# bdwsq1996/Effi-MVS-plus

Measured on NVIDIA B200. Metric: depth_maps_per_sec_1600x1184_5view, higher is better.
Workload: dtype hi+lo bf16 MMA x3, f32 accumulate (3-D regularization, fp32-grade) / f32 (warp, lookup, regression)

## Files before the change

effi-mvs-plus_b200/csrc/conv3d_tc.cu:

```cuda
#include <cuda_bf16.h>

#include <algorithm>
#include <cstdlib>
#include <cstring>
#include <vector>

#include "common.cuh"

namespace effimvs {
namespace {

constexpr int TILE_M = 128;
constexpr int SEG_VOX = 136;
constexpr int SEG_BYTES = SEG_VOX * 16;
constexpr int MAX_SEGS = 96;
constexpr int MAX_OPS = 160;
constexpr int MAX_BLOCKS = 56;
constexpr int MAX_PHASES = 8;
constexpr int ZSWEEP_R = 4;

enum { L_REG = 0, L_SPLIT = 1 };

struct ActLayout {
    int kind, planes, D, H, W;
// ... 352 lines not shown
            v = T.transposed ? w[((size_t)ci * T.cout + n) * 27 + tap] : w[((size_t)n * T.cin + ci) * 27 + tap];
        }
        __nv_bfloat16 hi = __float2bfloat16(v);
        dst[i] = lo ? __float2bfloat16(v - __bfloat162float(hi)) : hi;
    }
}

struct PackJobs { int n; PackTable T[8]; const float* w[8]; __nv_bfloat16* dst[8]; };
__global__ void pack_weights_multi_kernel(const __grid_constant__ PackJobs J) {
    const PackTable& T = J.T[blockIdx.y];
    const float* __restrict__ w = J.w[blockIdx.y];
    __nv_bfloat16* __restrict__ dst = J.dst[blockIdx.y];
    const int total = T.n_blocks * 2 * T.rows * 8;
    for (int i = blockIdx.x * blockDim.x + threadIdx.x; i < total; i += gridDim.x * blockDim.x) {
        const int kk = i & 7, row_all = (i >> 3) % T.rows, j = (i / (8 * T.rows)) & 1, blk = i / (16 * T.rows);
        const int row = T.stack > 1 ? row_all % T.brows : row_all;
        const bool lo = row >= T.N;
        const int n = lo ? row - T.N : row;
        const Block c = T.blk[blk];
        const int tap_bc = j ? c.tap1 : c.tap0, cb = j ? c.cb1 : c.cb0;
        const int tap = (T.stack > 1 && tap_bc >= 0) ? (T.stack - 1 - row_all / T.brows) * 9 + tap_bc : tap_bc;
        float v = 0.0f;
        if (tap >= 0 && n < T.cout) {
            const int ci = cb + kk;
            v = T.transposed ? w[((size_t)ci * T.cout + n) * 27 + tap] : w[((size_t)n * T.cin + ci) * 27 + tap];
        }
        __nv_bfloat16 hi = __float2bfloat16(v);
        dst[i] = lo ? __float2bfloat16(v - __bfloat162float(hi)) : hi;
    }
}

struct HaloJobs { int n; uint4* ptr[8]; ActLayout L[8]; int planes_before[9]; };
__global__ void zero_halo_kernel(const __grid_constant__ HaloJobs J, int B) {
    int job = 0;
    while (job + 1 < J.n && (int)blockIdx.x >= J.planes_before[job + 1]) ++job;
    const ActLayout& L = J.L[job];
    const int d = L.kind == L_SPLIT ? L.D / 2 : L.D, Pz = d + 2;
    const int local = blockIdx.x - J.planes_before[job];
    const int vol = local / Pz, zp = local - vol * Pz;
    uint4* __restrict__ base = J.ptr[job] + (long long)vol * L.vs;
    const uint4 zero = make_uint4(0, 0, 0, 0);
    const int tid = blockIdx.y * blockDim.x + threadIdx.x, nt = gridDim.y * blockDim.x;
    if (zp == 0) for (int i = tid; i < L.guard; i += nt) base[i] = zero;
    if (zp == Pz - 1) for (int i = tid; i < L.guard; i += nt) base[L.vs - L.guard + i] = zero;
    uint4* __restrict__ plane = base + L.guard + (long long)zp * L.zstride;
    if (zp == 0 || zp == Pz - 1) {
        for (int i = tid; i < (int)L.zstride; i += nt) plane[i] = zero;
    } else {
        for (int i = tid; i < L.Px; i += nt) { plane[i] = zero; plane[(long long)(L.Py - 1) * L.Px + i] = zero; }
        for (int y = 1 + tid; y < L.Py - 1; y += nt) { plane[(long long)y * L.Px] = zero; plane[(long long)y * L.Px + L.Px - 1] = zero; }
    }
}

constexpr int CIN1_X = 4;
template <int S>
__global__ void __launch_bounds__(128)
conv_cin1_kernel(const float* __restrict__ x, const float* __restrict__ w, const float* __restrict__ bias, int D, int H, int W,
                 const ActLayout OL, int plane, uint4* __restrict__ out) {
    __shared__ __align__(16) float sw[27 * 8 + 8];
    pdl_trigger();
    for (int i = threadIdx.x; i < 27 * 8; i += blockDim.x) sw[(i % 27) * 8 + i / 27] = w[i];
    if (threadIdx.x < 8) sw[216 + threadIdx.x] = bias[threadIdx.x];
    pdl_wait();
    __syncthreads();
    const int b = blockIdx.y;
    const int Ho = OL.H, Wo = OL.W;
    const int Wq = (Wo + CIN1_X - 1) / CIN1_X;
    const size_t o = (size_t)blockIdx.x * blockDim.x + threadIdx.x;
    if (o >= (size_t)D * Ho * Wq) return;
    const int ox0 = (int)(o % Wq) * CIN1_X, oy = (int)((o / Wq) % Ho), oz = (int)(o / ((size_t)Wq * Ho));
    constexpr int NIN = (CIN1_X - 1) * S + 3;
    float acc[CIN1_X][8];
#pragma unroll
    for (int i = 0; i < CIN1_X; ++i)
#pragma unroll
        for (int c = 0; c < 8; ++c) acc[i][c] = sw[216 + c];
    const float* xb = x + (size_t)b * D * H * W;
    const int ix0 = ox0 * S - 1;
#pragma unroll
    for (int a = 0; a < 3; ++a) {
        const int iz = oz + a - 1;
#pragma unroll
        for (int bb = 0; bb < 3; ++bb) {
            const int iy = oy * S + bb - 1;
            const bool row_ok = iz >= 0 && iz < D && iy >= 0 && iy < H;
            const float* row = xb + ((size_t)(row_ok ? iz : 0) * H + (row_ok ? iy : 0)) * W;
            float in[NIN];
#pragma unroll
            for (int j = 0; j < NIN; ++j) {
                const int ix = ix0 + j;
                in[j] = (row_ok && ix >= 0 && ix < W) ? __ldg(row + ix) : 0.0f;
            }
#pragma unroll
            for (int c = 0; c < 3; ++c) {
                const float4 w0 = *reinterpret_cast<const float4*>(sw + (a * 9 + bb * 3 + c) * 8);
                const float4 w1 = *reinterpret_cast<const float4*>(sw + (a * 9 + bb * 3 + c) * 8 + 4);
#pragma unroll
                for (int i = 0; i < CIN1_X; ++i) {
                    const float v = in[i * S + c];
                    acc[i][0] = fmaf(v, w0.x, acc[i][0]); acc[i][1] = fmaf(v, w0.y, acc[i][1]);
                    acc[i][2] = fmaf(v, w0.z, acc[i][2]); acc[i][3] = fmaf(v, w0.w, acc[i][3]);
                    acc[i][4] = fmaf(v, w1.x, acc[i][4]); acc[i][5] = fmaf(v, w1.y, acc[i][5]);
                    acc[i][6] = fmaf(v, w1.z, acc[i][6]); acc[i][7] = fmaf(v, w1.w, acc[i][7]);
                }
            }
        }
    }
#pragma unroll
    for (int i = 0; i < CIN1_X; ++i) {
        if (ox0 + i >= Wo) break;
#pragma unroll
        for (int j = 0; j < 8; ++j) acc[i][j] = fmaxf(acc[i][j], 0.0f);
        store_voxel(out, OL, b, plane, oz, oy, ox0 + i, acc[i]);
    }
}

__global__ void to_c8_kernel(const float* __restrict__ x, int C, const ActLayout L, uint4* __restrict__ out) {
    const int b = blockIdx.y;
    const int groups = (C + 7) / 8;
    const size_t vox = (size_t)L.D * L.H * L.W;
    const size_t o = (size_t)blockIdx.x * blockDim.x + threadIdx.x;
    if (o >= vox * groups) return;
    const int g = (int)(o / vox);
    const size_t r = o % vox;
    const int xx = (int)(r % L.W), yy = (int)((r / L.W) % L.H), zz = (int)(r / ((size_t)L.W * L.H));
    float v[8];
#pragma unroll
    for (int j = 0; j < 8; ++j) {
        const int c = g * 8 + j;
        v[j] = c < C ? x[((size_t)b * C + c) * vox + r] : 0.0f;
    }
    store_voxel(out, L, b, g, zz, yy, xx, v);
}
__global__ void from_c8_kernel(const uint4* __restrict__ in, int C, const ActLayout L, float* __restrict__ y) {
    const int b = blockIdx.y;
    const int groups = (C + 7) / 8;
    const size_t vox = (size_t)L.D * L.H * L.W;
    const size_t o = (size_t)blockIdx.x * blockDim.x + threadIdx.x;
    if (o >= vox * groups) return;
    const int g = (int)(o / vox);
    const size_t r = o % vox;
    const int xx = (int)(r % L.W), yy = (int)((r / L.W) % L.H), zz = (int)(r / ((size_t)L.W * L.H));
    float v[8];
    load_voxel(in, L, b, g, zz, yy, xx, v);
#pragma unroll
    for (int j = 0; j < 8; ++j) {
        const int c = g * 8 + j;
        if (c < C) y[((size_t)b * C + c) * vox + r] = v[j];
    }
}

struct Term { int seg, byte_off, tap, cls; };
struct PlaneSeg { long long off; int copy_vox; };

int pow2_cols(int n) { int c = 32; while (c < n) c <<= 1; return c; }

bool assemble(ConvProgram& P, PackTable& T, const std::vector<Term>& terms, const std::vector<PlaneSeg>& pseg, int NP,
              long long plane_stride, long long lo_plane_off, bool hilo) {
    const int SPP = (int)pseg.size();
    const int halves = hilo ? 2 : 1;
    const int n_phases = (hilo && NP == 4) ? 2 : 1;
    const int NPph = NP / n_phases;
    if (n_phases > MAX_PHASES) return false;
    P.n_phases = n_phases;
    P.b_rows = T.rows = hilo ? 2 * P.N : P.N;
    P.b_lbo_rows = P.b_rows; P.cls_z = 0; T.stack = 1; T.brows = T.rows;
// ... 243 lines not shown
int run_pack_multi(int n, const PackTable* T, const float* const* w, void* const* dst, cudaStream_t st) {
    static thread_local PackJobs J;
    J.n = n;
    int most = 0;
    for (int i = 0; i < n; ++i) {
        J.T[i] = T[i]; J.w[i] = w[i]; J.dst[i] = (__nv_bfloat16*)dst[i];
        most = std::max(most, T[i].n_blocks * 2 * T[i].rows * 8);
    }
    pack_weights_multi_kernel<<<dim3(ceil_div(most, 256), n), 256, 0, st>>>(J);
    return check_launch("pack_weights_multi_kernel");
}

int run_zero_halo(int n, void* const* ptr, const ActLayout* L, int B, cudaStream_t st) {
    static thread_local HaloJobs J;
    J.n = n;
    int total = 0;
    for (int i = 0; i < n; ++i) {
        J.ptr[i] = (uint4*)ptr[i]; J.L[i] = L[i];
        J.planes_before[i] = total;
        const int d = L[i].kind == L_SPLIT ? L[i].D / 2 : L[i].D;
        total += B * L[i].planes * (L[i].kind == L_SPLIT ? 8 : 1) * (d + 2);
    }
    J.planes_before[n] = total;
    zero_halo_kernel<<<dim3(total, 16), 128, 0, st>>>(J, B);
    return check_launch("zero_halo_kernel");
}

int run_tile_kernel(const ConvProgram& P, int B, const void* in, const ActLayout& IL, const void* wpk, const float* bias,
                    const ActLayout& OL, void* out, const ActLayout* RL, const void* res, float* out_f32, cudaStream_t st) {
    size_t smem = program_smem(P);
    EFFI_REQUIRE(smem <= 220 * 1024, EFFIMVS_EUNSUPPORTED, "conv_tc: tile needs %zu bytes of shared memory", smem);
    static bool attr_set = false;
    if (!attr_set) {
        cudaError_t e = cudaFuncSetAttribute(conv_tc_kernel, cudaFuncAttributeMaxDynamicSharedMemorySize, 220 * 1024);
        if (e != cudaSuccess) { set_error("conv_tc: cudaFuncSetAttribute: %s", cudaGetErrorString(e)); return EFFIMVS_ECUDA; }
        attr_set = true;
    }
    const int tiles_per_plane = ceil_div(P.gH * P.gPx, TILE_M);
    const long long n_tiles = (long long)tiles_per_plane * P.gD * B;
    EFFI_REQUIRE(n_tiles < (1ll << 31) && (long long)P.gPx * (P.gH + 2) < (1ll << 30), EFFIMVS_EUNSUPPORTED, "conv_tc: volume too large");
    int per_sm = (smem <= 110 * 1024 && P.tmem_cols <= 256) ? 2 : 1;
    if (const char* e = getenv("EFFIMVS_TC_MAXCTA")) {
        const int by_smem = (int)((227 * 1024) / (smem + 1024 + 4096)), by_tmem = 512 / P.tmem_cols;
        per_sm = std::max(1, std::min(atoi(e), std::min(by_smem, by_tmem)));
    }
    const int grid = (int)std::min<long long>(n_tiles, (long long)kNumSMs * per_sm);
    ActLayout rl = RL ? *RL : OL;
    if (const char* dbg = getenv("EFFIMVS_TC_DEBUG")) const_cast<ConvProgram&>(P).debug = atoi(dbg);
    launch_kernel(conv_tc_kernel, grid, dim3(CTA_THREADS), smem, st, P, (const uint4*)in, IL.batch_stride, (const uint8_t*)wpk, bias, OL, (uint4*)out, rl,
                                                    (const uint4*)res, out_f32, (int)n_tiles, tiles_per_plane);
    return check_launch("conv_tc_kernel");
}

int run_cin1(const float* x, const float* w, const float* bias, int B, int D, int H, int W, int s, const ActLayout& OL, int plane,
             void* out, cudaStream_t st) {
    size_t work = (size_t)D * OL.H * ((OL.W + CIN1_X - 1) / CIN1_X);
    dim3 grid((unsigned)((work + 127) / 128), B);
    if (s == 2) launch_kernel(conv_cin1_kernel<2>, grid, dim3(128), 0, st, x, w, bias, D, H, W, OL, plane, (uint4*)out);
    else launch_kernel(conv_cin1_kernel<1>, grid, dim3(128), 0, st, x, w, bias, D, H, W, OL, plane, (uint4*)out);
    return check_launch("conv_cin1_kernel");
}

template <bool RAW = false>
__device__ __forceinline__ void load_voxel_f32(const uint4* __restrict__ hi, long long lo_delta, long long idx, float (&v)[8]) {
    if (RAW) {
        const uint4 a = __ldg(hi + idx), c = __ldg(hi + idx + lo_delta);
        v[0] = __uint_as_float(a.x); v[1] = __uint_as_float(a.y); v[2] = __uint_as_float(a.z); v[3] = __uint_as_float(a.w);
        v[4] = __uint_as_float(c.x); v[5] = __uint_as_float(c.y); v[6] = __uint_as_float(c.z); v[7] = __uint_as_float(c.w);
        return;
    }
    unpack_bf16x8(__ldg(hi + idx), v);
    if (lo_delta) {
        float l[8];
        unpack_bf16x8(__ldg(hi + idx + lo_delta), l);
#pragma unroll
        for (int j = 0; j < 8; ++j) v[j] += l[j];
    }
}

constexpr int COUT1_X = 4;

template <bool RAW>
__global__ void __launch_bounds__(128)
conv_cout1_kernel(const uint4* __restrict__ in, const ActLayout IL, const float* __restrict__ w, const float* __restrict__ bias, int relu,
                  float* __restrict__ out) {
    __shared__ __align__(16) float sw[27 * 8];
    pdl_trigger();
    for (int i = threadIdx.x; i < 27 * 8; i += blockDim.x) sw[(i % 27) * 8 + i / 27] = w[i];
    pdl_wait();
    __syncthreads();
    const int b = blockIdx.y, D = IL.D, H = IL.H, W = IL.W;
    const int Wq = (W + COUT1_X - 1) / COUT1_X;
    const size_t o = (size_t)blockIdx.x * blockDim.x + threadIdx.x;
    if (o >= (size_t)D * H * Wq) return;
    const int x0 = (int)(o % Wq) * COUT1_X, y = (int)((o / Wq) % H), z = (int)(o / ((size_t)Wq * H));
    const long long lo_delta = (long long)IL.lo_off * IL.vs;
    const long long base = (long long)b * IL.batch_stride + IL.guard;
    float acc[COUT1_X];
#pragma unroll
    for (int i = 0; i < COUT1_X; ++i) acc[i] = bias ? __ldg(bias) : 0.0f;
#pragma unroll
    for (int a = 0; a < 3; ++a)
#pragma unroll
        for (int bb = 0; bb < 3; ++bb) {
            const long long row = base + (long long)(z + a) * IL.zstride + (long long)(y + bb) * IL.Px + x0;
            float v[COUT1_X + 2][8];
#pragma unroll
            for (int j = 0; j < COUT1_X + 2; ++j) {
                if (x0 + j <= W + 1) load_voxel_f32<RAW>(in, lo_delta, row + j, v[j]);
                else {
#pragma unroll
                    for (int c = 0; c < 8; ++c) v[j][c] = 0.0f;
                }
            }
#pragma unroll
            for (int c = 0; c < 3; ++c) {
                const float4 w0 = *reinterpret_cast<const float4*>(sw + (a * 9 + bb * 3 + c) * 8);
                const float4 w1 = *reinterpret_cast<const float4*>(sw + (a * 9 + bb * 3 + c) * 8 + 4);
#pragma unroll
                for (int i = 0; i < COUT1_X; ++i) {
                    const float (&u)[8] = v[i + c];
                    float t = acc[i];
                    t = fmaf(u[0], w0.x, t); t = fmaf(u[1], w0.y, t); t = fmaf(u[2], w0.z, t); t = fmaf(u[3], w0.w, t);
                    t = fmaf(u[4], w1.x, t); t = fmaf(u[5], w1.y, t); t = fmaf(u[6], w1.z, t); t = fmaf(u[7], w1.w, t);
                    acc[i] = t;
                }
            }
        }
    float* op = out + (((size_t)b * D + z) * H + y) * W + x0;
#pragma unroll
    for (int i = 0; i < COUT1_X; ++i)
        if (x0 + i < W) op[i] = relu ? fmaxf(acc[i], 0.0f) : acc[i];
}

template <bool RAW>
__global__ void __launch_bounds__(128)
deconv_cout1_kernel(const uint4* __restrict__ in, const ActLayout IL, const float* __restrict__ w, const float* __restrict__ bias, int relu,
                    float* __restrict__ out) {
    __shared__ __align__(16) float sw[27 * 8];
    pdl_trigger();
    for (int i = threadIdx.x; i < 27 * 8; i += blockDim.x) sw[(i % 27) * 8 + i / 27] = w[i];
    pdl_wait();
    __syncthreads();
    const int b = blockIdx.y, D = IL.D, H = IL.H, W = IL.W;
    const size_t o = (size_t)blockIdx.x * blockDim.x + threadIdx.x;
    if (o >= (size_t)D * H * W) return;
    const int x = (int)(o % W), y = (int)((o / W) % H), z = (int)(o / ((size_t)W * H));
    const long long lo_delta = (long long)IL.lo_off * IL.vs;
    const long long base = (long long)b * IL.batch_stride + IL.guard;
    const float b0 = bias ? __ldg(bias) : 0.0f;
    float acc[2][2] = {{b0, b0}, {b0, b0}};
    {
        const bool last = (threadIdx.x & 31) == 31 || x == W - 1;
#pragma unroll
        for (int a = 0; a < 3; ++a)
#pragma unroll
            for (int dy = 0; dy < 2; ++dy) {
                const uint4* p = in + base + (long long)(z + 2 - a) * IL.zstride + (long long)(y + 1 + dy) * IL.Px + (x + 1);
                asm volatile("prefetch.global.L1 [%0];" ::"l"(p));
                if (RAW || lo_delta) asm volatile("prefetch.global.L1 [%0];" ::"l"(p + lo_delta));
                if (last) {
                    asm volatile("prefetch.global.L1 [%0];" ::"l"(p + 1));
                    if (RAW || lo_delta) asm volatile("prefetch.global.L1 [%0];" ::"l"(p + 1 + lo_delta));
                }
            }
    }
    float v[3][2][2][8];
#pragma unroll
    for (int a = 0; a < 3; ++a) {
        const long long plane = base + (long long)(z + 2 - a) * IL.zstride;
#pragma unroll
        for (int dy = 0; dy < 2; ++dy)
#pragma unroll
            for (int dx = 0; dx < 2; ++dx) load_voxel_f32<RAW>(in, lo_delta, plane + (long long)(y + 1 + dy) * IL.Px + (x + 1 + dx), v[a][dy][dx]);
    }
#pragma unroll
    for (int a = 0; a < 3; ++a) {
#pragma unroll
        for (int bb = 0; bb < 3; ++bb)
#pragma unroll
            for (int c = 0; c < 3; ++c) {
                const int py = bb != 1, dy = bb == 0, px = c != 1, dx = c == 0;
                const float4 w0 = *reinterpret_cast<const float4*>(sw + (a * 9 + bb * 3 + c) * 8);
                const float4 w1 = *reinterpret_cast<const float4*>(sw + (a * 9 + bb * 3 + c) * 8 + 4);
                const float (&u)[8] = v[a][dy][dx];
                float t = acc[py][px];
                t = fmaf(u[0], w0.x, t); t = fmaf(u[1], w0.y, t); t = fmaf(u[2], w0.z, t); t = fmaf(u[3], w0.w, t);
                t = fmaf(u[4], w1.x, t); t = fmaf(u[5], w1.y, t); t = fmaf(u[6], w1.z, t); t = fmaf(u[7], w1.w, t);
                acc[py][px] = t;
            }
    }
    const int Ho = 2 * H, Wo = 2 * W;
#pragma unroll
    for (int py = 0; py < 2; ++py) {
        float2 r = make_float2(acc[py][0], acc[py][1]);
        if (relu) { r.x = fmaxf(r.x, 0.0f); r.y = fmaxf(r.y, 0.0f); }
        *reinterpret_cast<float2*>(out + (((size_t)b * D + z) * Ho + 2 * y + py) * Wo + 2 * x) = r;
    }
}

int run_cout1(bool deconv, int B, const void* in, const ActLayout& IL, const float* w, const float* bias, int relu, float* out,
              cudaStream_t st, bool raw_f32 = false) {
    if (deconv) {
        const size_t work = (size_t)IL.D * IL.H * IL.W;
        const dim3 grid((unsigned)((work + 127) / 128), B);
        if (raw_f32) launch_kernel(deconv_cout1_kernel<true>, grid, dim3(128), 0, st, (const uint4*)in, IL, w, bias, relu, out);
        else launch_kernel(deconv_cout1_kernel<false>, grid, dim3(128), 0, st, (const uint4*)in, IL, w, bias, relu, out);
        return check_launch("deconv_cout1_kernel");
    }
    const size_t work = (size_t)IL.D * IL.H * ((IL.W + COUT1_X - 1) / COUT1_X);
    const dim3 grid((unsigned)((work + 127) / 128), B);
    if (raw_f32) launch_kernel(conv_cout1_kernel<true>, grid, dim3(128), 0, st, (const uint4*)in, IL, w, bias, relu, out);
    else launch_kernel(conv_cout1_kernel<false>, grid, dim3(128), 0, st, (const uint4*)in, IL, w, bias, relu, out);
    return check_launch("conv_cout1_kernel");
}

struct Carver {
    char* base; size_t off, cap;
    void* take(size_t bytes) { void* p = base ? base + off : nullptr; off += (bytes + 255) & ~(size_t)255; return p; }
};

constexpr size_t W_SLOT = 128 * 1024;

}

size_t costreg_bf16_workspace_bytes(int B, int D, int H, int W, bool hilo) {
    ActLayout c0 = make_layout(L_REG, 8, D, H, W, hilo), c1 = make_layout(L_SPLIT, 8, D, H, W, hilo);
    ActLayout c2 = make_layout(L_REG, 16, D / 2, H / 2, W / 2, hilo), c3 = make_layout(L_SPLIT, 16, D / 2, H / 2, W / 2, hilo);
    ActLayout c4 = make_layout(L_REG, 32, D / 4, H / 4, W / 4, hilo);
    return layout_bytes(c0, B) * 2 + layout_bytes(c1, B) + layout_bytes(c2, B) * 2 + layout_bytes(c3, B) + layout_bytes(c4, B) * 2 +
           8 * W_SLOT + 4096;
}

int costreg_bf16(const float* x, const float* const* weights, const float* const* biases, int B, int D, int H, int W, bool hilo,
                 int phases, void* ws, size_t ws_bytes, float* prob_out, cudaStream_t st) {
    EFFI_REQUIRE(D % 4 == 0 && H % 4 == 0 && W % 4 == 0, EFFIMVS_EUNSUPPORTED, "costreg bf16: D, H, W must be multiples of 4");
    EFFI_REQUIRE(D <= 65535 && B <= 65535, EFFIMVS_EUNSUPPORTED, "costreg bf16: D or B too large");
    const int D2 = D / 2, H2 = H / 2, W2 = W / 2, D4 = D / 4, H4 = H / 4, W4 = W / 4;
    ActLayout L0 = make_layout(L_REG, 8, D, H, W, hilo), L1 = make_layout(L_SPLIT, 8, D, H, W, hilo);
    ActLayout L2 = make_layout(L_REG, 16, D2, H2, W2, hilo), L3 = make_layout(L_SPLIT, 16, D2, H2, W2, hilo);
    ActLayout L4 = make_layout(L_REG, 32, D4, H4, W4, hilo), L5 = L4, L6 = L2, L7 = L0;
    Carver cv{(char*)ws, 0, ws_bytes};
    void* c0 = cv.take(layout_bytes(L0, B)); void* c7 = cv.take(layout_bytes(L7, B)); void* c1 = cv.take(layout_bytes(L1, B));
    void* c2 = cv.take(layout_bytes(L2, B)); void* c6 = cv.take(layout_bytes(L6, B)); void* c3 = cv.take(layout_bytes(L3, B));
    void* c4 = cv.take(layout_bytes(L4, B)); void* c5 = cv.take(layout_bytes(L5, B));
    const size_t act_bytes = cv.off;
    void* wp[8];
    for (int i = 0; i < 8; ++i) wp[i] = cv.take(W_SLOT);
    EFFI_REQUIRE(cv.off <= ws_bytes, EFFIMVS_EWORKSPACE, "costreg bf16: workspace %zu < %zu", ws_bytes, cv.off);
    (void)act_bytes;
    int rc;
    const bool prepare = (phases & EFFIMVS_WS_PREPARE) != 0, run = (phases & EFFIMVS_WS_RUN) != 0;
    if (prepare) {
        void* bufs[8] = {c0, c7, c1, c2, c6, c3, c4, c5};
        ActLayout lays[8] = {L0, L7, L1, L2, L6, L3, L4, L5};
        if ((rc = run_zero_halo(8, bufs, lays, B, st))) return rc;
    }

    static thread_local ConvProgram P[8];
    static thread_local PackTable T[8];
    bool ok = build_conv_s1(P[0], T[0], 8, 8, L0, 1) && build_conv_s2(P[1], T[1], 8, 16, L1, 1) &&
              build_conv_s1(P[2], T[2], 16, 16, L2, 1) && build_conv_s2(P[3], T[3], 16, 32, L3, 1) &&
              build_conv_s1(P[4], T[4], 32, 32, L4, 1) && build_deconv(P[5], T[5], 32, 16, L5, 2, 1) &&
              build_deconv(P[6], T[6], 16, 8, L6, 2, 1) && build_conv_s1(P[7], T[7], 8, 1, L7, 0);
    EFFI_REQUIRE(ok, EFFIMVS_EUNSUPPORTED, "costreg bf16: program does not fit");
    for (int i = 0; i < 8; ++i)
        EFFI_REQUIRE(program_weight_bytes(T[i]) <= W_SLOT, EFFIMVS_EUNSUPPORTED, "costreg bf16: packed weights of layer %d too large", i + 1);
    if (prepare && (rc = run_pack_multi(8, T, weights + 1, wp, st))) return rc;
    if (!run) return EFFIMVS_OK;
    if ((rc = run_cin1(x, weights[0], biases[0], B, D, H, W, 1, L0, 0, c0, st))) return rc;
    if ((rc = run_tile_kernel(P[0], B, c0, L0, wp[0], biases[1], L1, c1, nullptr, nullptr, nullptr, st))) return rc;
    if ((rc = run_tile_kernel(P[1], B, c1, L1, wp[1], biases[2], L2, c2, nullptr, nullptr, nullptr, st))) return rc;
    if ((rc = run_tile_kernel(P[2], B, c2, L2, wp[2], biases[3], L3, c3, nullptr, nullptr, nullptr, st))) return rc;
    if ((rc = run_tile_kernel(P[3], B, c3, L3, wp[3], biases[4], L4, c4, nullptr, nullptr, nullptr, st))) return rc;
    if ((rc = run_tile_kernel(P[4], B, c4, L4, wp[4], biases[5], L5, c5, nullptr, nullptr, nullptr, st))) return rc;
    if ((rc = run_tile_kernel(P[5], B, c5, L5, wp[5], biases[6], L6, c6, &L3, c3, nullptr, st))) return rc;
    const char* prob_path = getenv("EFFIMVS_PROB_PATH");
    const bool raw_prob = hilo && prob_path && !strcmp(prob_path, "raw");
    P[6].out_f32_pair = raw_prob ? 1 : 0;
    if ((rc = run_tile_kernel(P[6], B, c6, L6, wp[6], biases[7], L7, c7, &L1, c1, nullptr, st))) return rc;
    if (raw_prob) return run_cout1(false, B, c7, L7, weights[8], nullptr, 0, prob_out, st, true);
    if (getenv("EFFIMVS_CUDA_CORE_PROB")) return run_cout1(false, B, c7, L7, weights[8], nullptr, 0, prob_out, st);
    return run_tile_kernel(P[7], B, c7, L7, wp[7], nullptr, L7, nullptr, nullptr, nullptr, prob_out, st);
}

size_t cost_up_bf16_workspace_bytes(int B, int D, int H, int W, bool hilo) {
    ActLayout cat = make_layout(L_REG, 16, D, H / 2, W / 2, hilo), c1 = make_layout(L_REG, 8, D, H / 2, W / 2, hilo);
    return layout_bytes(cat, B) + layout_bytes(c1, B) + 2 * W_SLOT + 4096;
}

int cost_up_bf16(const float* x, const float* prev, const float* const* weights, const float* const* biases, int B, int D, int H,
                 int W, bool hilo, int phases, void* ws, size_t ws_bytes, float* out, cudaStream_t st) {
    EFFI_REQUIRE(D <= 65535 && B <= 65535, EFFIMVS_EUNSUPPORTED, "cost_up bf16: D or B too large");
    const int H2 = H / 2, W2 = W / 2;
    ActLayout Lcat = make_layout(L_REG, 16, D, H2, W2, hilo), L1 = make_layout(L_REG, 8, D, H2, W2, hilo);
    Carver cv{(char*)ws, 0, ws_bytes};
    void* cat = cv.take(layout_bytes(Lcat, B)); void* c1 = cv.take(layout_bytes(L1, B));
    const size_t act_bytes = cv.off;
    void* wp1 = cv.take(W_SLOT); void* wp2 = cv.take(W_SLOT);
    EFFI_REQUIRE(cv.off <= ws_bytes, EFFIMVS_EWORKSPACE, "cost_up bf16: workspace %zu < %zu", ws_bytes, cv.off);
    (void)act_bytes;
    int rc;
    const bool prepare = (phases & EFFIMVS_WS_PREPARE) != 0, run = (phases & EFFIMVS_WS_RUN) != 0;
    if (prepare) {
        void* bufs[2] = {cat, c1};
        ActLayout lays[2] = {Lcat, L1};
        if ((rc = run_zero_halo(2, bufs, lays, B, st))) return rc;
    }
    static thread_local ConvProgram P1, P2;
    static thread_local PackTable T12[2];
    PackTable &T1 = T12[0], &T2 = T12[1];
    bool ok = build_conv_s1(P1, T1, 16, 8, Lcat, 1) && build_deconv(P2, T2, 8, 1, L1, 1, 1);
    EFFI_REQUIRE(ok, EFFIMVS_EUNSUPPORTED, "cost_up bf16: program does not fit");
    if (prepare) {
        void* dsts[2] = {wp1, wp2};
        if ((rc = run_pack_multi(2, T12, weights + 2, dsts, st))) return rc;
    }
    if (!run) return EFFIMVS_OK;
    if ((rc = run_cin1(x, weights[0], biases[0], B, D, H, W, 2, Lcat, 0, cat, st))) return rc;
    if ((rc = run_cin1(prev, weights[1], biases[1], B, D, H2, W2, 1, Lcat, 1, cat, st))) return rc;
    const bool tc_cout1 = getenv("EFFIMVS_TC_COUT1") != nullptr;
    const bool raw = hilo && !tc_cout1 && !getenv("EFFIMVS_NO_RAW_F32");
    P1.out_f32_pair = raw ? 1 : 0;
    if ((rc = run_tile_kernel(P1, B, cat, Lcat, wp1, biases[2], L1, c1, nullptr, nullptr, nullptr, st))) return rc;
    ActLayout LO = make_layout(L_REG, 8, D, H, W, false);
    if (!tc_cout1) return run_cout1(true, B, c1, L1, weights[3], biases[3], 1, out, st, raw);
    return run_tile_kernel(P2, B, c1, L1, wp2, biases[3], LO, nullptr, nullptr, nullptr, out, st);
}

size_t conv3d_bf16_workspace_bytes(int B, int Cin, int Cout, int D, int H, int W, int sd, int transposed, bool hilo) {
    int Do = D, Ho = H, Wo = W;
    if (transposed) { Do = D * sd; Ho = H * 2; Wo = W * 2; }
    else if (sd == 2) { Do = D / 2; Ho = H / 2; Wo = W / 2; }
    ActLayout LI = make_layout(!transposed && sd == 2 ? L_SPLIT : L_REG, (Cin + 7) / 8 * 8, D, H, W, hilo);
    ActLayout LO = make_layout(L_REG, (Cout + 7) / 8 * 8, Do, Ho, Wo, hilo);
    return layout_bytes(LI, B) + 2 * layout_bytes(LO, B) + W_SLOT + 4096;
}

int conv3d_bf16(const float* x, const float* weight, const float* bias, const float* residual, int B, int Cin, int Cout, int D,
                int H, int W, int sd, int transposed, int relu, bool hilo, void* ws, size_t ws_bytes, float* y, cudaStream_t st) {
    EFFI_REQUIRE((Cin == 8 || Cin == 16 || Cin == 32) && Cout >= 1 && Cout <= 32, EFFIMVS_EUNSUPPORTED,
                 "conv3d_bf16: Cin in {8,16,32}, Cout <= 32");
    int Do = D, Ho = H, Wo = W;
    if (transposed) { Do = D * sd; Ho = H * 2; Wo = W * 2; }
    else if (sd == 2) { EFFI_REQUIRE(D % 2 == 0 && H % 2 == 0 && W % 2 == 0, EFFIMVS_EUNSUPPORTED, "conv3d_bf16: stride 2 needs even dims"); Do = D / 2; Ho = H / 2; Wo = W / 2; }
    const int Cop = (Cout + 7) / 8 * 8;
    ActLayout LI = make_layout(!transposed && sd == 2 ? L_SPLIT : L_REG, Cin, D, H, W, hilo);
    ActLayout LO = make_layout(L_REG, Cop, Do, Ho, Wo, hilo);
    Carver cv{(char*)ws, 0, ws_bytes};
    void* xin = cv.take(layout_bytes(LI, B)); void* yout = cv.take(layout_bytes(LO, B)); void* rin = cv.take(layout_bytes(LO, B));
    const size_t act_bytes = cv.off;
    void* wp = cv.take(W_SLOT);
    EFFI_REQUIRE(cv.off <= ws_bytes, EFFIMVS_EWORKSPACE, "conv3d_bf16: workspace %zu < %zu", ws_bytes, cv.off);
    if (cudaMemsetAsync(ws, 0, act_bytes, st) != cudaSuccess) { set_error("conv3d_bf16: memset failed"); return EFFIMVS_ECUDA; }
    static thread_local ConvProgram P;
    static thread_local PackTable T;
    bool ok = transposed ? build_deconv(P, T, Cin, Cout, LI, sd, relu) : (sd == 2 ? build_conv_s2(P, T, Cin, Cout, LI, relu) : build_conv_s1(P, T, Cin, Cout, LI, relu));
    EFFI_REQUIRE(ok && program_weight_bytes(T) <= W_SLOT, EFFIMVS_EUNSUPPORTED, "conv3d_bf16: program does not fit");
    int rc;
    if ((rc = run_pack(T, weight, wp, st))) return rc;
    size_t n_in = (size_t)D * H * W * (Cin / 8), n_out = (size_t)Do * Ho * Wo * (Cop / 8);
    to_c8_kernel<<<dim3((unsigned)((n_in + 255) / 256), B), 256, 0, st>>>(x, Cin, LI, (uint4*)xin);
    if (residual) to_c8_kernel<<<dim3((unsigned)((n_out + 255) / 256), B), 256, 0, st>>>(residual, Cout, LO, (uint4*)rin);
    if ((rc = check_launch("to_c8_kernel"))) return rc;
    if ((rc = run_tile_kernel(P, B, xin, LI, wp, bias, LO, yout, residual ? &LO : nullptr, residual ? rin : nullptr, nullptr, st))) return rc;
    from_c8_kernel<<<dim3((unsigned)((n_out + 255) / 256), B), 256, 0, st>>>((const uint4*)yout, Cout, LO, y);
    return check_launch("from_c8_kernel");
}

}

extern "C" size_t effimvs_conv3d_bf16_workspace_bytes(int B, int Cin, int Cout, int D, int H, int W, int sd, int transposed, int precision) {
    return effimvs::conv3d_bf16_workspace_bytes(B, Cin, Cout, D, H, W, sd, transposed, precision == EFFIMVS_PREC_BF16X3);
// ... 11 lines not shown
```

Baseline: 165.7.

## Tile thin Cin=1 conv and Cout=1 deconv kernels with shared-memory z-ring reuse

Rewrites the single-input-channel conv kernel as a 2-D tiled kernel that sweeps along depth, staging input planes into a four-slot shared-memory ring with cp.async. Each loaded plane is reused across three output depths and neighbouring pixels instead of being re-read from global memory. Accumulation uses packed f32x2 FMAs, and the two cost_up cin1 launches are fused into one kernel that writes both planes. The Cout=1 deconv gets the same z-ring treatment with register-staged prefetch of the next plane, in exchange for more shared memory, a barrier per depth step, and fewer CTAs per SM.

```diff
diff --git a/effi-mvs-plus_b200/csrc/conv3d_tc.cu b/effi-mvs-plus_b200/csrc/conv3d_tc.cu
--- a/effi-mvs-plus_b200/csrc/conv3d_tc.cu
+++ b/effi-mvs-plus_b200/csrc/conv3d_tc.cu
@@ -428,66 +428,153 @@
     }
 }
 
-constexpr int CIN1_X = 4;
+constexpr int THIN_THREADS = 128;
+constexpr int THIN_RING = 4;
+
+int thin_zrun(int tiles, int B, int D) {
+    const int runs = std::min(D, std::max(1, ceil_div(4 * kNumSMs, tiles * B)));
+    return ceil_div(D, runs);
+}
+
+typedef unsigned long long pk2;
+__device__ __forceinline__ pk2 pk(float lo, float hi) { pk2 r; asm("mov.b64 %0, {%1, %2};" : "=l"(r) : "f"(lo), "f"(hi)); return r; }
+__device__ __forceinline__ void unpk(pk2 v, float& lo, float& hi) { asm("mov.b64 {%0, %1}, %2;" : "=f"(lo), "=f"(hi) : "l"(v)); }
+__device__ __forceinline__ void fma2_acc(pk2& acc, pk2 a, pk2 b) { asm("fma.rn.f32x2 %0, %1, %2, %0;" : "+l"(acc) : "l"(a), "l"(b)); }
+
+constexpr int CIN_TX = 64, CIN_TY = 8, CIN_PX = 4;
+static_assert(CIN_TX / CIN_PX * CIN_TY == THIN_THREADS, "one output row segment per thread");
 template <int S>
-__global__ void __launch_bounds__(128)
-conv_cin1_kernel(const float* __restrict__ x, const float* __restrict__ w, const float* __restrict__ bias, int D, int H, int W,
-                 const ActLayout OL, int plane, uint4* __restrict__ out) {
-    __shared__ __align__(16) float sw[27 * 8 + 8];
-    pdl_trigger();
-    for (int i = threadIdx.x; i < 27 * 8; i += blockDim.x) sw[(i % 27) * 8 + i / 27] = w[i];
-    if (threadIdx.x < 8) sw[216 + threadIdx.x] = bias[threadIdx.x];
-    pdl_wait();
-    __syncthreads();
-    const int b = blockIdx.y;
-    const int Ho = OL.H, Wo = OL.W;
-    const int Wq = (Wo + CIN1_X - 1) / CIN1_X;
-    const size_t o = (size_t)blockIdx.x * blockDim.x + threadIdx.x;
-    if (o >= (size_t)D * Ho * Wq) return;
-    const int ox0 = (int)(o % Wq) * CIN1_X, oy = (int)((o / Wq) % Ho), oz = (int)(o / ((size_t)Wq * Ho));
-    constexpr int NIN = (CIN1_X - 1) * S + 3;
-    float acc[CIN1_X][8];
-#pragma unroll
-    for (int i = 0; i < CIN1_X; ++i)
-#pragma unroll
-        for (int c = 0; c < 8; ++c) acc[i][c] = sw[216 + c];
-    const float* xb = x + (size_t)b * D * H * W;
-    const int ix0 = ox0 * S - 1;
-#pragma unroll
+struct CinRows {
+    static constexpr int ROWS = (CIN_TY - 1) * S + 3;
+    static constexpr int COLS = ((CIN_TX - 1) * S + 3 + 3) / 4 * 4;
+    static constexpr int PLANE = ROWS * COLS;
+    static constexpr int PER_THREAD = (PLANE + THIN_THREADS - 1) / THIN_THREADS;
+    static constexpr int NIN = (CIN_PX - 1) * S + 3;
+};
+
+template <int S>
+__device__ __forceinline__ void cin_stage(float* __restrict__ slot, const float* __restrict__ xb, int D, int H, int W, int z, int gy0,
+                                          int gx0) {
+    using R = CinRows<S>;
+    const bool zok = z >= 0 && z < D;
+    const float* __restrict__ pl = xb + (size_t)(zok ? z : 0) * H * W;
+#pragma unroll
+    for (int i = 0; i < R::PER_THREAD; ++i) {
+        const int e = threadIdx.x + i * THIN_THREADS;
+        if (e >= R::PLANE) break;
+        const int row = e / R::COLS, col = e - row * R::COLS;
+        const int gy = gy0 + row, gx = gx0 + col;
+        const bool ok = zok && gy >= 0 && gy < H && gx >= 0 && gx < W;
+        const float* src = ok ? pl + (size_t)gy * W + gx : pl;
+        asm volatile("cp.async.ca.shared.global [%0], [%1], 4, %2;" ::"r"(smem_u32(slot + e)), "l"(src), "r"(ok ? 4 : 0) : "memory");
+    }
+}
+__device__ __forceinline__ void cp_async_wait_all() { asm volatile("cp.async.wait_all;" ::: "memory"); }
+
+template <int S>
+__device__ __forceinline__ void cin_compute(const float* __restrict__ ring, int oz, const float* __restrict__ sw, int ty, int tx,
+                                            float (&res)[CIN_PX][8]) {
+    using R = CinRows<S>;
+    pk2 acc[CIN_PX][4];
+#pragma unroll
+    for (int i = 0; i < CIN_PX; ++i)
+#pragma unroll
+        for (int c = 0; c < 4; ++c) acc[i][c] = pk(sw[216 + 2 * c], sw[217 + 2 * c]);
+#pragma unroll 1
     for (int a = 0; a < 3; ++a) {
-        const int iz = oz + a - 1;
-#pragma unroll
+        const float* __restrict__ slot = ring + ((oz + a - 1 + THIN_RING) % THIN_RING) * R::PLANE;
+#pragma unroll 1
         for (int bb = 0; bb < 3; ++bb) {
-            const int iy = oy * S + bb - 1;
-            const bool row_ok = iz >= 0 && iz < D && iy >= 0 && iy < H;
-            const float* row = xb + ((size_t)(row_ok ? iz : 0) * H + (row_ok ? iy : 0)) * W;
-            float in[NIN];
-#pragma unroll
-            for (int j = 0; j < NIN; ++j) {
-                const int ix = ix0 + j;
-                in[j] = (row_ok && ix >= 0 && ix < W) ? __ldg(row + ix) : 0.0f;
-            }
+            const float* __restrict__ row = slot + (ty * S + bb) * R::COLS + tx * CIN_PX * S;
+            float in[R::NIN];
+#pragma unroll
+            for (int j = 0; j + 4 <= R::NIN; j += 4) {
+                const float4 q = *reinterpret_cast<const float4*>(row + j);
+                in[j] = q.x; in[j + 1] = q.y; in[j + 2] = q.z; in[j + 3] = q.w;
+            }
+#pragma unroll
+            for (int j = R::NIN / 4 * 4; j < R::NIN; ++j) in[j] = row[j];
 #pragma unroll
             for (int c = 0; c < 3; ++c) {
                 const float4 w0 = *reinterpret_cast<const float4*>(sw + (a * 9 + bb * 3 + c) * 8);
                 const float4 w1 = *reinterpret_cast<const float4*>(sw + (a * 9 + bb * 3 + c) * 8 + 4);
-#pragma unroll
-                for (int i = 0; i < CIN1_X; ++i) {
+                const pk2 w01 = pk(w0.x, w0.y), w23 = pk(w0.z, w0.w), w45 = pk(w1.x, w1.y), w67 = pk(w1.z, w1.w);
+#pragma unroll
+                for (int i = 0; i < CIN_PX; ++i) {
                     const float v = in[i * S + c];
-                    acc[i][0] = fmaf(v, w0.x, acc[i][0]); acc[i][1] = fmaf(v, w0.y, acc[i][1]);
-                    acc[i][2] = fmaf(v, w0.z, acc[i][2]); acc[i][3] = fmaf(v, w0.w, acc[i][3]);
-                    acc[i][4] = fmaf(v, w1.x, acc[i][4]); acc[i][5] = fmaf(v, w1.y, acc[i][5]);
-                    acc[i][6] = fmaf(v, w1.z, acc[i][6]); acc[i][7] = fmaf(v, w1.w, acc[i][7]);
+                    const pk2 vv = pk(v, v);
+                    fma2_acc(acc[i][0], vv, w01); fma2_acc(acc[i][1], vv, w23);
+                    fma2_acc(acc[i][2], vv, w45); fma2_acc(acc[i][3], vv, w67);
                 }
             }
         }
     }
 #pragma unroll
-    for (int i = 0; i < CIN1_X; ++i) {
-        if (ox0 + i >= Wo) break;
-#pragma unroll
-        for (int j = 0; j < 8; ++j) acc[i][j] = fmaxf(acc[i][j], 0.0f);
-        store_voxel(out, OL, b, plane, oz, oy, ox0 + i, acc[i]);
+    for (int i = 0; i < CIN_PX; ++i)
+#pragma unroll
+        for (int c = 0; c < 4; ++c) {
+            unpk(acc[i][c], res[i][2 * c], res[i][2 * c + 1]);
+            res[i][2 * c] = fmaxf(res[i][2 * c], 0.0f);
+            res[i][2 * c + 1] = fmaxf(res[i][2 * c + 1], 0.0f);
+        }
+}
+
+template <int S0, bool TWO>
+__global__ void __launch_bounds__(THIN_THREADS, 4)
+conv_cin1_kernel(const float* __restrict__ x0, const float* __restrict__ w0, const float* __restrict__ b0, int H0, int W0,
+                 const float* __restrict__ x1, const float* __restrict__ w1, const float* __restrict__ b1, int D, int zrun,
+                 const ActLayout OL, uint4* __restrict__ out) {
+    using R0 = CinRows<S0>;
+    using R1 = CinRows<1>;
+    constexpr int NL = TWO ? 2 : 1;
+    __shared__ __align__(16) float sw[NL][27 * 8 + 8];
+    __shared__ __align__(16) float s0[THIN_RING * R0::PLANE];
+    __shared__ __align__(16) float s1[TWO ? THIN_RING * R1::PLANE : 4];
+    pdl_trigger();
+    for (int i = threadIdx.x; i < 27 * 8; i += THIN_THREADS) {
+        sw[0][(i % 27) * 8 + i / 27] = w0[i];
+        if (TWO) sw[NL - 1][(i % 27) * 8 + i / 27] = w1[i];
+    }
+    if (threadIdx.x < 8) {
+        sw[0][216 + threadIdx.x] = b0[threadIdx.x];
+        if (TWO) sw[NL - 1][216 + threadIdx.x] = b1[threadIdx.x];
+    }
+    pdl_wait();
+    const int Ho = OL.H, Wo = OL.W, b = blockIdx.z;
+    const int tiles_x = ceil_div(Wo, CIN_TX);
+    const int ox_t = (blockIdx.x % tiles_x) * CIN_TX, oy_t = (blockIdx.x / tiles_x) * CIN_TY;
+    const int z0 = blockIdx.y * zrun, z1 = min(D, z0 + zrun);
+    const int tx = threadIdx.x % (CIN_TX / CIN_PX), ty = threadIdx.x / (CIN_TX / CIN_PX);
+    const int oy = oy_t + ty, ox = ox_t + tx * CIN_PX;
+    const bool active = oy < Ho && ox < Wo;
+    const float* __restrict__ xb0 = x0 + (size_t)b * D * H0 * W0;
+    const float* __restrict__ xb1 = TWO ? x1 + (size_t)b * D * Ho * Wo : nullptr;
+    for (int iz = z0 - 1; iz <= z0 + 1; ++iz) {
+        cin_stage<S0>(s0 + ((iz + THIN_RING) % THIN_RING) * R0::PLANE, xb0, D, H0, W0, iz, oy_t * S0 - 1, ox_t * S0 - 1);
+        if (TWO) cin_stage<1>(s1 + ((iz + THIN_RING) % THIN_RING) * R1::PLANE, xb1, D, Ho, Wo, iz, oy_t - 1, ox_t - 1);
+    }
+    cp_async_wait_all();
+    __syncthreads();
+    for (int oz = z0; oz < z1; ++oz) {
+        if (oz + 2 <= z1) {
+            cin_stage<S0>(s0 + ((oz + 2) % THIN_RING) * R0::PLANE, xb0, D, H0, W0, oz + 2, oy_t * S0 - 1, ox_t * S0 - 1);
+            if (TWO) cin_stage<1>(s1 + ((oz + 2) % THIN_RING) * R1::PLANE, xb1, D, Ho, Wo, oz + 2, oy_t - 1, ox_t - 1);
+        }
+        if (active) {
+            float res[CIN_PX][8];
+            cin_compute<S0>(s0, oz, sw[0], ty, tx, res);
+#pragma unroll
+            for (int i = 0; i < CIN_PX; ++i)
+                if (ox + i < Wo) store_voxel(out, OL, b, 0, oz, oy, ox + i, res[i]);
+            if (TWO) {
+                cin_compute<1>(s1, oz, sw[NL - 1], ty, tx, res);
+#pragma unroll
+                for (int i = 0; i < CIN_PX; ++i)
+                    if (ox + i < Wo) store_voxel(out, OL, b, 1, oz, oy, ox + i, res[i]);
+            }
+        }
+        cp_async_wait_all();
+        __syncthreads();
     }
 }
 
@@ -837,12 +924,18 @@
     return check_launch("conv_tc_kernel");
 }
 
-int run_cin1(const float* x, const float* w, const float* bias, int B, int D, int H, int W, int s, const ActLayout& OL, int plane,
-             void* out, cudaStream_t st) {
-    size_t work = (size_t)D * OL.H * ((OL.W + CIN1_X - 1) / CIN1_X);
-    dim3 grid((unsigned)((work + 127) / 128), B);
-    if (s == 2) launch_kernel(conv_cin1_kernel<2>, grid, dim3(128), 0, st, x, w, bias, D, H, W, OL, plane, (uint4*)out);
-    else launch_kernel(conv_cin1_kernel<1>, grid, dim3(128), 0, st, x, w, bias, D, H, W, OL, plane, (uint4*)out);
+int run_cin1(const float* x, const float* w, const float* bias, int H, int W, int s, const float* prev, const float* wp,
+             const float* bp, int B, const ActLayout& OL, void* out, cudaStream_t st) {
+    const int D = OL.D, tiles = ceil_div(OL.W, CIN_TX) * ceil_div(OL.H, CIN_TY), zrun = thin_zrun(tiles, B, D);
+    const dim3 grid(tiles, ceil_div(D, zrun), B);
+    if (prev && s == 2)
+        launch_kernel(conv_cin1_kernel<2, true>, grid, dim3(THIN_THREADS), 0, st, x, w, bias, H, W, prev, wp, bp, D, zrun, OL, (uint4*)out);
+    else if (!prev && s == 1)
+        launch_kernel(conv_cin1_kernel<1, false>, grid, dim3(THIN_THREADS), 0, st, x, w, bias, H, W, prev, wp, bp, D, zrun, OL, (uint4*)out);
+    else {
+        set_error("conv_cin1: no kernel for stride %d with%s a second input", s, prev ? "" : "out");
+        return EFFIMVS_EUNSUPPORTED;
+    }
     return check_launch("conv_cin1_kernel");
 }
 
@@ -918,79 +1011,146 @@
         if (x0 + i < W) op[i] = relu ? fmaxf(acc[i], 0.0f) : acc[i];
 }
 
+constexpr int DC_TX = 64, DC_TY = 4;
+static_assert(DC_TY * 32 == THIN_THREADS && DC_TX == 64, "a warp per input row, two positions per lane");
+constexpr int DC_ROWS = DC_TY + 1, DC_COLS = DC_TX + 1, DC_VOX = DC_ROWS * DC_COLS;
+constexpr int DC_PER_THREAD = (DC_VOX + THIN_THREADS - 1) / THIN_THREADS;
+
 template <bool RAW>
-__global__ void __launch_bounds__(128)
+__device__ __forceinline__ void dc_fetch(const uint4* __restrict__ plane, long long lo_delta, const ActLayout& IL, int y_t, int x_t,
+                                         uint4 (&hi)[DC_PER_THREAD], uint4 (&lo)[DC_PER_THREAD]) {
+#pragma unroll
+    for (int i = 0; i < DC_PER_THREAD; ++i) {
+        const int e = threadIdx.x + i * THIN_THREADS;
+        const int r = e / DC_COLS, c = e - r * DC_COLS;
+        const int yp = y_t + 1 + r, xp = x_t + 1 + c;
+        const bool ok = e < DC_VOX && yp <= IL.H + 1 && xp <= IL.W + 1;
+        const long long idx = (long long)yp * IL.Px + xp;
+        hi[i] = ok ? __ldg(plane + idx) : make_uint4(0, 0, 0, 0);
+        lo[i] = ok && (RAW || lo_delta) ? __ldg(plane + idx + lo_delta) : make_uint4(0, 0, 0, 0);
+    }
+}
+template <bool RAW>
+__device__ __forceinline__ void dc_put(float4* __restrict__ slot, long long lo_delta, const uint4 (&hi)[DC_PER_THREAD],
+                                       const uint4 (&lo)[DC_PER_THREAD]) {
+#pragma unroll
+    for (int i = 0; i < DC_PER_THREAD; ++i) {
+        const int e = threadIdx.x + i * THIN_THREADS;
+        if (e >= DC_VOX) break;
+        const int r = e / DC_COLS, c = e - r * DC_COLS;
+        float4 q0, q1;
+        if (RAW) {
+            q0 = make_float4(__uint_as_float(hi[i].x), __uint_as_float(hi[i].y), __uint_as_float(hi[i].z), __uint_as_float(hi[i].w));
+            q1 = make_float4(__uint_as_float(lo[i].x), __uint_as_float(lo[i].y), __uint_as_float(lo[i].z), __uint_as_float(lo[i].w));
+        } else {
+            float v[8];
+            unpack_bf16x8(hi[i], v);
+            if (lo_delta) {
+                float l[8];
+                unpack_bf16x8(lo[i], l);
+#pragma unroll
+                for (int j = 0; j < 8; ++j) v[j] += l[j];
+            }
+            q0 = make_float4(v[0], v[1], v[2], v[3]);
+            q1 = make_float4(v[4], v[5], v[6], v[7]);
+        }
+        slot[(r * 2 + 0) * DC_COLS + c] = q0;
+        slot[(r * 2 + 1) * DC_COLS + c] = q1;
+    }
+}
+
+template <bool RAW>
+__global__ void __launch_bounds__(THIN_THREADS)
 deconv_cout1_kernel(const uint4* __restrict__ in, const ActLayout IL, const float* __restrict__ w, const float* __restrict__ bias, int relu,
-                    float* __restrict__ out) {
-    __shared__ __align__(16) float sw[27 * 8];
+                    int zrun, float* __restrict__ out) {
+    __shared__ __align__(16) float sw[27 * 8 + 4];
+    __shared__ __align__(16) float4 ring[THIN_RING * DC_ROWS * 2 * DC_COLS];
     pdl_trigger();
-    for (int i = threadIdx.x; i < 27 * 8; i += blockDim.x) sw[(i % 27) * 8 + i / 27] = w[i];
+    for (int i = threadIdx.x; i < 27 * 8; i += THIN_THREADS) sw[(i % 27) * 8 + i / 27] = w[i];
+    if (threadIdx.x == 0) sw[216] = bias ? bias[0] : 0.0f;
     pdl_wait();
+    const int b = blockIdx.z, D = IL.D, H = IL.H, W = IL.W;
+    const int tiles_x = ceil_div(W, DC_TX);
+    const int x_t = (blockIdx.x % tiles_x) * DC_TX, y_t = (blockIdx.x / tiles_x) * DC_TY;
+    const int z0 = blockIdx.y * zrun, z1 = min(D, z0 + zrun);
+    const int lane = threadIdx.x & 31, ty = threadIdx.x >> 5;
+    const int y = y_t + ty;
+    const long long lo_delta = (long long)IL.lo_off * IL.vs;
+    const uint4* __restrict__ base = in + (long long)b * IL.batch_stride + IL.guard;
+    constexpr int SLOT = DC_ROWS * 2 * DC_COLS;
+    uint4 hi[DC_PER_THREAD], lo[DC_PER_THREAD];
+    for (int zp = z0; zp <= z0 + 2; ++zp) {
+        dc_fetch<RAW>(base + (long long)zp * IL.zstride, lo_delta, IL, y_t, x_t, hi, lo);
+        dc_put<RAW>(ring + (zp % THIN_RING) * SLOT, lo_delta, hi, lo);
+    }
     __syncthreads();
-    const int b = blockIdx.y, D = IL.D, H = IL.H, W = IL.W;
-    const size_t o = (size_t)blockIdx.x * blockDim.x + threadIdx.x;
-    if (o >= (size_t)D * H * W) return;
-    const int x = (int)(o % W), y = (int)((o / W) % H), z = (int)(o / ((size_t)W * H));
-    const long long lo_delta = (long long)IL.lo_off * IL.vs;
-    const long long base = (long long)b * IL.batch_stride + IL.guard;
-    const float b0 = bias ? __ldg(bias) : 0.0f;
-    float acc[2][2] = {{b0, b0}, {b0, b0}};
-    {
-        const bool last = (threadIdx.x & 31) == 31 || x == W - 1;
-#pragma unroll
-        for (int a = 0; a < 3; ++a)
-#pragma unroll
-            for (int dy = 0; dy < 2; ++dy) {
-                const uint4* p = in + base + (long long)(z + 2 - a) * IL.zstride + (long long)(y + 1 + dy) * IL.Px + (x + 1);
-                asm volatile("prefetch.global.L1 [%0];" ::"l"(p));
-                if (RAW || lo_delta) asm volatile("prefetch.global.L1 [%0];" ::"l"(p + lo_delta));
-                if (last) {
-                    asm volatile("prefetch.global.L1 [%0];" ::"l"(p + 1));
-                    if (RAW || lo_delta) asm volatile("prefetch.global.L1 [%0];" ::"l"(p + 1 + lo_delta));
+    const int Ho = 2 * H, Wo = 2 * W;
+    for (int z = z0; z < z1; ++z) {
+        const bool more = z + 2 <= z1;
+        if (more) dc_fetch<RAW>(base + (long long)(z + 3) * IL.zstride, lo_delta, IL, y_t, x_t, hi, lo);
+        if (y < H) {
+            const float b0 = sw[216];
+            float acc[2][2][2];
+#pragma unroll
+            for (int p = 0; p < 2; ++p)
+#pragma unroll
+                for (int py = 0; py < 2; ++py) acc[p][py][0] = acc[p][py][1] = b0;
+#pragma unroll
+            for (int a = 0; a < 3; ++a) {
+                const float4* __restrict__ slot = ring + ((z + 2 - a) % THIN_RING) * SLOT;
+                float v[2][2][2][8];
+#pragma unroll
+                for (int p = 0; p < 2; ++p)
+#pragma unroll
+                    for (int dy = 0; dy < 2; ++dy)
+#pragma unroll
+                        for (int dx = 0; dx < 2; ++dx) {
+                            const int col = lane + 32 * p + dx;
+                            const float4 q0 = slot[((ty + dy) * 2 + 0) * DC_COLS + col], q1 = slot[((ty + dy) * 2 + 1) * DC_COLS + col];
+                            float (&u)[8] = v[p][dy][dx];
+                            u[0] = q0.x; u[1] = q0.y; u[2] = q0.z; u[3] = q0.w; u[4] = q1.x; u[5] = q1.y; u[6] = q1.z; u[7] = q1.w;
+                        }
+#pragma unroll
+                for (int bb = 0; bb < 3; ++bb)
+#pragma unroll
+                    for (int c = 0; c < 3; ++c) {
+                        const int py = bb != 1, dy = bb == 0, px = c != 1, dx = c == 0;
+                        const float4 w0 = *reinterpret_cast<const float4*>(sw + (a * 9 + bb * 3 + c) * 8);
+                        const float4 w1 = *reinterpret_cast<const float4*>(sw + (a * 9 + bb * 3 + c) * 8 + 4);
+#pragma unroll
+                        for (int p = 0; p < 2; ++p) {
+                            const float (&u)[8] = v[p][dy][dx];
+                            float t = acc[p][py][px];
+                            t = fmaf(u[0], w0.x, t); t = fmaf(u[1], w0.y, t); t = fmaf(u[2], w0.z, t); t = fmaf(u[3], w0.w, t);
+                            t = fmaf(u[4], w1.x, t); t = fmaf(u[5], w1.y, t); t = fmaf(u[6], w1.z, t); t = fmaf(u[7], w1.w, t);
+                            acc[p][py][px] = t;
+                        }
+                    }
+            }
+#pragma unroll
+            for (int p = 0; p < 2; ++p) {
+                const int x = x_t + lane + 32 * p;
+                if (x >= W) continue;
+#pragma unroll
+                for (int py = 0; py < 2; ++py) {
+                    float2 r = make_float2(acc[p][py][0], acc[p][py][1]);
+                    if (relu) { r.x = fmaxf(r.x, 0.0f); r.y = fmaxf(r.y, 0.0f); }
+                    *reinterpret_cast<float2*>(out + (((size_t)b * D + z) * Ho + 2 * y + py) * Wo + 2 * x) = r;
                 }
             }
-    }
-    float v[3][2][2][8];
-#pragma unroll
-    for (int a = 0; a < 3; ++a) {
-        const long long plane = base + (long long)(z + 2 - a) * IL.zstride;
-#pragma unroll
-        for (int dy = 0; dy < 2; ++dy)
-#pragma unroll
-            for (int dx = 0; dx < 2; ++dx) load_voxel_f32<RAW>(in, lo_delta, plane + (long long)(y + 1 + dy) * IL.Px + (x + 1 + dx), v[a][dy][dx]);
-    }
-#pragma unroll
-    for (int a = 0; a < 3; ++a) {
-#pragma unroll
-        for (int bb = 0; bb < 3; ++bb)
-#pragma unroll
-            for (int c = 0; c < 3; ++c) {
-                const int py = bb != 1, dy = bb == 0, px = c != 1, dx = c == 0;
-                const float4 w0 = *reinterpret_cast<const float4*>(sw + (a * 9 + bb * 3 + c) * 8);
-                const float4 w1 = *reinterpret_cast<const float4*>(sw + (a * 9 + bb * 3 + c) * 8 + 4);
-                const float (&u)[8] = v[a][dy][dx];
-                float t = acc[py][px];
-                t = fmaf(u[0], w0.x, t); t = fmaf(u[1], w0.y, t); t = fmaf(u[2], w0.z, t); t = fmaf(u[3], w0.w, t);
-                t = fmaf(u[4], w1.x, t); t = fmaf(u[5], w1.y, t); t = fmaf(u[6], w1.z, t); t = fmaf(u[7], w1.w, t);
-                acc[py][px] = t;
-            }
-    }
-    const int Ho = 2 * H, Wo = 2 * W;
-#pragma unroll
-    for (int py = 0; py < 2; ++py) {
-        float2 r = make_float2(acc[py][0], acc[py][1]);
-        if (relu) { r.x = fmaxf(r.x, 0.0f); r.y = fmaxf(r.y, 0.0f); }
-        *reinterpret_cast<float2*>(out + (((size_t)b * D + z) * Ho + 2 * y + py) * Wo + 2 * x) = r;
+        }
+        if (more) dc_put<RAW>(ring + ((z + 3) % THIN_RING) * SLOT, lo_delta, hi, lo);
+        __syncthreads();
     }
 }
 
 int run_cout1(bool deconv, int B, const void* in, const ActLayout& IL, const float* w, const float* bias, int relu, float* out,
               cudaStream_t st, bool raw_f32 = false) {
     if (deconv) {
-        const size_t work = (size_t)IL.D * IL.H * IL.W;
-        const dim3 grid((unsigned)((work + 127) / 128), B);
-        if (raw_f32) launch_kernel(deconv_cout1_kernel<true>, grid, dim3(128), 0, st, (const uint4*)in, IL, w, bias, relu, out);
-        else launch_kernel(deconv_cout1_kernel<false>, grid, dim3(128), 0, st, (const uint4*)in, IL, w, bias, relu, out);
+        const int tiles = ceil_div(IL.W, DC_TX) * ceil_div(IL.H, DC_TY), zrun = thin_zrun(tiles, B, IL.D);
+        const dim3 grid(tiles, ceil_div(IL.D, zrun), B);
+        if (raw_f32) launch_kernel(deconv_cout1_kernel<true>, grid, dim3(THIN_THREADS), 0, st, (const uint4*)in, IL, w, bias, relu, zrun, out);
+        else launch_kernel(deconv_cout1_kernel<false>, grid, dim3(THIN_THREADS), 0, st, (const uint4*)in, IL, w, bias, relu, zrun, out);
         return check_launch("deconv_cout1_kernel");
     }
     const size_t work = (size_t)IL.D * IL.H * ((IL.W + COUT1_X - 1) / COUT1_X);
@@ -1053,7 +1213,7 @@
         EFFI_REQUIRE(program_weight_bytes(T[i]) <= W_SLOT, EFFIMVS_EUNSUPPORTED, "costreg bf16: packed weights of layer %d too large", i + 1);
     if (prepare && (rc = run_pack_multi(8, T, weights + 1, wp, st))) return rc;
     if (!run) return EFFIMVS_OK;
-    if ((rc = run_cin1(x, weights[0], biases[0], B, D, H, W, 1, L0, 0, c0, st))) return rc;
+    if ((rc = run_cin1(x, weights[0], biases[0], H, W, 1, nullptr, nullptr, nullptr, B, L0, c0, st))) return rc;
     if ((rc = run_tile_kernel(P[0], B, c0, L0, wp[0], biases[1], L1, c1, nullptr, nullptr, nullptr, st))) return rc;
     if ((rc = run_tile_kernel(P[1], B, c1, L1, wp[1], biases[2], L2, c2, nullptr, nullptr, nullptr, st))) return rc;
     if ((rc = run_tile_kernel(P[2], B, c2, L2, wp[2], biases[3], L3, c3, nullptr, nullptr, nullptr, st))) return rc;
@@ -1102,8 +1262,7 @@
         if ((rc = run_pack_multi(2, T12, weights + 2, dsts, st))) return rc;
     }
     if (!run) return EFFIMVS_OK;
-    if ((rc = run_cin1(x, weights[0], biases[0], B, D, H, W, 2, Lcat, 0, cat, st))) return rc;
-    if ((rc = run_cin1(prev, weights[1], biases[1], B, D, H2, W2, 1, Lcat, 1, cat, st))) return rc;
+    if ((rc = run_cin1(x, weights[0], biases[0], H, W, 2, prev, weights[1], biases[1], B, Lcat, cat, st))) return rc;
     const bool tc_cout1 = getenv("EFFIMVS_TC_COUT1") != nullptr;
     const bool raw = hilo && !tc_cout1 && !getenv("EFFIMVS_NO_RAW_F32");
     P1.out_f32_pair = raw ? 1 : 0;
```

After: 166.1 (median of 6 runs). About the same (+0.2%).
